# Enigmatisms/AdaPT

Measured on AMD Instinct MI355X. Metric: Msamples/s (W*H*spp/s), unidirectional MIS path tracing, higher is better.
Workload: dtype f32

## Files before the change

adapt_amd/_lib.py:

```python
from __future__ import annotations

import ctypes as C
import os

_HERE = os.path.dirname(os.path.abspath(__file__))
LIB_PATHS = {"fast": os.environ.get("ADAPT_MI_LIB") or os.path.join(_HERE, "libadapt_mi.so"),
             "exact": os.environ.get("ADAPT_MI_LIB_EXACT") or os.path.join(_HERE, "libadapt_mi_exact.so")}
_variant = "exact" if os.environ.get("APT_EXACT", "0") not in ("", "0") else "fast"
LIB_PATH = LIB_PATHS[_variant]

f32p = C.POINTER(C.c_float)
i32p = C.POINTER(C.c_int32)
u32p = C.POINTER(C.c_uint32)
u8p = C.POINTER(C.c_uint8)
f64p = C.POINTER(C.c_double)
APT_N_KERNELS = 5
KERNEL_NAMES = ("generate", "extend", "shade", "shadow", "finalize")


class AptError(RuntimeError):
    pass


class SceneDesc(C.Structure):
# ... 67 lines not shown
    "apt_get_stats": (C.c_int, [C.c_void_p, C.POINTER(Stats)]),
    "apt_device_ptr": (C.c_int, [C.c_void_p, C.POINTER(C.c_void_p), i32p]),
    "apt_stream": (C.c_int, [C.c_void_p, C.POINTER(C.c_void_p)]),
    "apt_intersect": (C.c_int, [C.c_void_p, C.c_int32, f32p, f32p, i32p, f32p, f32p]),
    "apt_occluded": (C.c_int, [C.c_void_p, C.c_int32, f32p, f32p, f32p, i32p]),
    "apt_rng_stream": (C.c_int, [C.c_int32, C.c_uint32, C.c_uint32, C.c_uint32, C.c_int32, u32p]),
    "apt_bxdf_probe": (C.c_int, [C.c_int32, C.c_int32, i32p, f32p, f32p, C.c_float, C.c_int32, C.c_uint32, f32p]),
    "apt_medium_probe": (C.c_int, [C.c_int32, C.c_int32, i32p, f32p, C.c_int32, f32p, C.c_uint32, f32p]),
    "apt_volume_probe": (C.c_int, [C.c_int32, C.c_int32, i32p, f32p, f32p, C.c_int32, f32p, C.c_uint32, f32p]),
    "apt_emitter_probe": (C.c_int, [C.c_void_p, C.c_int32, f32p, C.c_uint32, f32p]),
    "apt_texture_probe": (C.c_int, [C.c_void_p, C.c_int32, i32p, f32p, f32p]),
    "apt_surface_maps_probe": (C.c_int, [C.c_void_p, C.c_int32, i32p, f32p, f32p]),
    "apt_transient_bin_probe": (C.c_int, [C.c_int32, C.c_int32, f32p, C.c_float, C.c_float, C.c_int32, i32p]),
    "apt_renderer_info": (C.c_int, [C.c_void_p, i32p, i32p, C.POINTER(C.c_int64), i32p, C.POINTER(C.c_char_p), i32p]),
    "apt_renderer_camera_fused": (C.c_int, [C.c_void_p, i32p]),
    "apt_measure_sclk_mhz": (C.c_int, [C.c_int32, f32p]),
    "apt_last_error": (C.c_char_p, []),
    "apt_version": (C.c_char_p, []),
}

_libs = {}


def use(variant: str) -> str:
    global _variant, LIB_PATH
    if variant not in LIB_PATHS:
        raise ValueError(f"unknown build variant {variant!r}")
    prev, _variant = _variant, variant
    LIB_PATH = LIB_PATHS[variant]
    return prev
# ... 36 lines not shown
```

adapt_amd/csrc/api.hip:

```cpp
#include <hip/hip_runtime.h>
#include <chrono>

#include <algorithm>
#include <cmath>
#include <cstdio>
#include <cstdlib>
#include <cstring>
#include <limits>
#include <memory>
#include <string>
#include <vector>

#include "../../include/adapt_mi.h"
#include "bvh_build.hpp"
#include "shade_stage.hpp"
#include "unit_kernels.hpp"
#include "volumetric.hpp"

#define APT_EXPORT extern "C" __attribute__((visibility("default")))

static thread_local std::string g_err;
static int fail(int code, const std::string& msg) { g_err = msg; return code; }
#define HIP_TRY(expr)                                                                              \
    do {                                                                                           \
// ... 164 lines not shown

enum Pipeline { PIPE_STAGED, PIPE_SORTED, PIPE_TRACED, PIPE_VOLUMETRIC };

struct apt_renderer {
    const apt_scene* scene = nullptr;
    apt_render_cfg cfg{};
    Params par{};
    int n_cols = 0, npix = 0, spp_batch = 1;
    int cnt = 0;
    std::vector<Lane> lanes;
    int n_lanes = 1;
    hipStream_t stream() const { return lanes[0].stream; }
    DevBuf accum, scratch, pix_key;
    DevBuf cam_strips;
    int camera_fuse = 0;
    Counters host_counters{};
    int grid_small = 0, grid_trace = 0, nq = APT_MAX_NQ;
    const ShadeVariant* shade = nullptr;
    int trace_mode = TRACE_BVH;
    int trace_nt = BLOCK;
    int trace_items = BLOCK;
    Pipeline pipeline = PIPE_STAGED;
    int dyn_fetch = 0;
    bool tile_ok = false;
    extend_fn extend = nullptr, fix = nullptr;
    int ovf_levels = 0;
    int n_cq = 0;
    int vev_single = 0;
    vev_shade_fn vev_all = nullptr;
    bool vev_live[APT_MAX_CLASSES] = {};
// ... 458 lines not shown
    }
    r->spp_batch = B;
    const int S = c.num_shadow_ray;
    const size_t subcap = subcap_of(B), cap = subcap * nq;
    if (cap >= (1ull << 31)) { return fail(APT_E_INVALID, "apt_renderer_create: batch too large (spp_per_batch * pixels must stay below 2^31)"); }
    Params& p = r->par;
    memcpy(p.cam_r, c.cam_r, sizeof(p.cam_r)); memcpy(p.cam_t, c.cam_t, sizeof(p.cam_t));
    p.inv_focal = c.inv_focal; p.half_w = c.half_w; p.half_h = c.half_h;
    p.W = c.width; p.H = c.height; p.n_cols = r->n_cols; p.npix = r->npix;
    p.band_width = c.band_width; p.rank = c.rank; p.world = c.world_size;
    p.do_crop = c.do_crop; p.sx = c.start_x; p.ex = c.end_x; p.sy = c.start_y; p.ey = c.end_y;
    p.max_bounce = c.max_bounce; p.S = S; p.inv_S = (S > 0) ? 1.f / (float)S : 1.f;
    p.use_rr = c.use_rr; p.use_mis = c.use_mis; p.anti_alias = c.anti_alias; p.stratified = c.stratified; p.two_sides = c.brdf_two_sides;
    p.rr_bounce_th = c.rr_bounce_th; p.rr_threshold = c.rr_threshold; p.seed = c.seed; p.cap = (uint32_t)cap; p.subcap = (uint32_t)subcap; p.nq = r->nq;
    p.inv_ns = 1.f / (float)sc->n_sources; p.inv_ns1 = (sc->n_sources > 1) ? 1.f / (float)(sc->n_sources - 1) : 1.f;
    p.volumetric_flat = c.volumetric ? 1 : 0; p.fix_par = 0;
    p.pix_bits = 0; while ((1u << p.pix_bits) < (uint32_t)r->npix) p.pix_bits++;
    if (((uint64_t)B << p.pix_bits) > (1ull << 32)) { return fail(APT_E_INVALID, "apt_renderer_create: spp_per_batch x pixels does not fit the 32-bit path id"); }
    std::vector<uint32_t> key((size_t)r->npix);
    for (int lp = 0; lp < r->npix; lp++) {
        const int lc = lp / c.height, j = lp % c.height, lb = lc / c.band_width, w_ = lc % c.band_width;
        const int i = (lb * c.world_size + c.rank) * c.band_width + w_;
        key[(size_t)lp] = (uint32_t)(i * c.height + j);
    }
    hipError_t e_ = upload(r->pix_key, key);
    if (e_ != hipSuccess) { return fail(APT_E_HIP, std::string("upload pix_key: ") + hipGetErrorString(e_)); }
    p.pix_key = r->pix_key.as<uint32_t>();
    return APT_OK;
}

static int small_scene_sweep(const apt_renderer* r) { return (r->tile_ok && r->scene->max_obj_prims >= APT_SWEEP_LIST_MIN) ? TRACE_TILE : TRACE_SWEEP; }
// ... 82 lines not shown
    cf.inv_focal = c.inv_focal; cf.half_w = c.half_w; cf.half_h = c.half_h;
    cf.width = c.width; cf.height = c.height; cf.n_cols = owned_columns(c); cf.band_width = c.band_width; cf.rank = c.rank; cf.world = c.world_size;
    return cf;
}
static int make_camera_strips(apt_renderer* r) {
    if (r->pipeline != PIPE_TRACED) return APT_OK;
    const apt_scene* sc = r->scene;
    const bool cull = !(getenv("APT_CAMERA_CULL") && atoi(getenv("APT_CAMERA_CULL")) == 0);
    std::vector<uint64_t> masks;
    if (apt::camera_strips(sc->h_prims.data(), sc->n_prims, sc->h_flat_recs, sc->h_flat_tab, sc->h_flat_counts, cam_film(r->cfg), cull, masks) != 0)
        return fail(APT_E_INVALID, "apt_renderer_create: camera strip lists: bad record or film");
    hipError_t e = upload(r->cam_strips, masks);
    if (e != hipSuccess) return fail(APT_E_HIP, std::string("upload camera strip lists: ") + hipGetErrorString(e));
    const bool want = !(getenv("APT_CAMERA_FUSE") && atoi(getenv("APT_CAMERA_FUSE")) == 0);
    r->camera_fuse = (want && !r->adaptive && !r->par.do_crop && r->par.max_bounce >= 1 && r->shade->traced_cam != nullptr) ? 1 : 0;
    return APT_OK;
}

APT_EXPORT int apt_camera_strips(const float* prims, int32_t n_prims, const int32_t* obj_info, int32_t n_objects, const apt_render_cfg* cfg, int32_t cull,
                                 uint64_t* masks, int32_t masks_cap, int32_t* n_strips, int32_t* n_pairs) {
    if (!prims || !obj_info || !cfg || n_prims <= 0 || n_objects <= 0 || !n_strips || !n_pairs) return fail(APT_E_INVALID, "apt_camera_strips: bad argument");
    apt_render_cfg c = *cfg;
    if (c.world_size <= 0) { c.world_size = 1; c.rank = 0; }
    if (c.band_width <= 0) c.band_width = c.width;
    if (c.width <= 0 || c.height <= 0 || c.rank < 0 || c.rank >= c.world_size || owned_columns(c) <= 0) return fail(APT_E_INVALID, "apt_camera_strips: bad film or rank");
    std::vector<float> st, tb; int cn[7];
    if (apt::build_flat(prims, n_prims, obj_info, n_objects, nullptr, st, tb, cn) != 0) return fail(APT_E_INVALID, "apt_camera_strips: obj_info range outside the primitive array");
    std::vector<uint64_t> m;
    if (apt::camera_strips(prims, n_prims, st, tb, cn, cam_film(c), cull != 0, m) != 0) return fail(APT_E_INVALID, "apt_camera_strips: bad record or film");
    *n_strips = (int32_t)m.size();
// ... 406 lines not shown
static int render_surface(apt_renderer* r, int32_t n_spp) {
    const DevScene& sc = r->scene->dev;
    const int nq = r->nq;
    int done = 0, batch = 0;
    hipEvent_t prev_fin = nullptr;
    const int batch_cap = lane_batch(r, n_spp);
    while (done < n_spp) {
        const int B = (n_spp - done < batch_cap) ? (n_spp - done) : batch_cap;
        Lane& ln = r->lanes[(size_t)(batch % r->n_lanes)];
        hipStream_t st = ln.stream;
        const Queues& q = ln.q;
        Counters* cnt = ln.cnt();
        Params p = r->par; p.cnt_base = r->cnt; p.spp_batch = B;
        const size_t total = (size_t)r->npix * (size_t)B;
        if (int rc = begin_batch(r, ln)) return rc;
#if APT_FAST
        if (r->pipeline == PIPE_TRACED) {
            const unsigned long long* strips = r->cam_strips.as<unsigned long long>();
            int cur = 0, b0 = 0;
            if (r->camera_fuse) {
                { LaunchTimer t(r, APT_K_SHADE, st); hipLaunchKernelGGL(r->shade->traced_cam, dim3(grid_for(total, r->grid_small, nq)), dim3(BLOCK), 0, st, sc, p, q, cnt, strips); }
                { LaunchTimer t(r, APT_K_SHADE, st); hipLaunchKernelGGL(r->shade->traced, dim3(r->grid_fix), dim3(BLOCK), 0, st, sc, p, q, cnt, 0, 0); }
                cur = 1; b0 = 1;
            } else {
                LaunchTimer t(r, APT_K_GENERATE, st);
                if (r->adaptive) hipLaunchKernelGGL(k_generate_trace_ad, dim3(grid_for(total, r->grid_small, 1)), dim3(BLOCK), 0, st, sc, p, q, cnt, (const uint8_t*)r->aq.active, strips);
                else hipLaunchKernelGGL(k_generate_trace, dim3(grid_for(total, r->grid_small, 1)), dim3(BLOCK), 0, st, sc, p, q, cnt, strips);
            }
            for (int b = b0; b < p.max_bounce; b++) {
                { LaunchTimer t(r, APT_K_SHADE, st); hipLaunchKernelGGL(r->shade->traced, dim3(grid_for(total, r->grid_small, nq)), dim3(BLOCK), 0, st, sc, p, q, cnt, cur, b); }
// ... 422 lines not shown
    }
    std::vector<unsigned long long> h((size_t)n_waves * 2);
    HIP_TRY(hipMemcpy(h.data(), out.p, h.size() * 8, hipMemcpyDeviceToHost));
    std::vector<double> r;
    for (int w = 0; w < n_waves; w++) if (h[2 * (size_t)w + 1] > 0) r.push_back(100.0 * (double)h[2 * (size_t)w] / (double)h[2 * (size_t)w + 1]);
    if (r.empty()) return fail(APT_E_STATE, "apt_measure_sclk_mhz: the wall clock did not advance");
    std::nth_element(r.begin(), r.begin() + r.size() / 2, r.end());
    *mhz = (float)r[r.size() / 2];
    return APT_OK;
}
APT_EXPORT int apt_renderer_camera_fused(const apt_renderer* r, int32_t* out) {
    if (!r || !out) return fail(APT_E_INVALID, "apt_renderer_camera_fused: null argument");
    *out = r->camera_fuse;
    return APT_OK;
}
APT_EXPORT int apt_renderer_info(const apt_renderer* r, int32_t* spp_batch, int32_t* n_subqueues, int64_t* queue_bytes, int32_t* lds_bytes, const char** shade_variant, int32_t* trace_mode) {
    if (!r) return fail(APT_E_INVALID, "apt_renderer_info: null handle");
    if (spp_batch) *spp_batch = r->spp_batch;
    if (n_subqueues) *n_subqueues = r->nq;
    if (queue_bytes) *queue_bytes = (int64_t)r->lanes[0].pool.bytes * (int64_t)r->lanes.size();
    if (lds_bytes) *lds_bytes = (int32_t)r->lds_bytes;
    if (shade_variant) *shade_variant = r->shade_name.c_str();
    if (trace_mode) *trace_mode = r->trace_mode;
    return APT_OK;
}
```

adapt_amd/csrc/shade_stage.hpp:

```cpp
#pragma once
#include "stages.hpp"

APT_D float ti_fmod(float a, float b) { float q = floorf(a / b); return a - b * q; }
APT_D f3 mix3(f3 a, f3 b, float t) { return a * (1.0f - t) + b * t; }
APT_D f3 texture_query(const DevScene& sc, int map, int obj, float u, float v) {
    const int* ti_ = sc.tex_i + 15 * obj + 5 * map; const float* tf = sc.tex_f + 6 * obj + 2 * map;
    const float w = (float)ti_[3], h = (float)ti_[4];
    const float scaled_u = ti_fmod((u * tf[0]) * w, w - 1.f), scaled_v = ti_fmod((v * tf[1]) * h, h - 1.f);
    float floor_u = floorf(scaled_u), floor_v = floorf(scaled_v);
    const float ratio_u = fmaxf(scaled_u - floor_u, 0.f), ratio_v = fmaxf(scaled_v - floor_v, 0.f);
    floor_u = fminf(fmaxf(floor_u, 0.f), w - 1.f); floor_v = fminf(fmaxf(floor_v, 0.f), h - 1.f);
    const float ceil_u = fminf(floor_u + 1.f, w - 1.f), ceil_v = fminf(floor_v + 1.f, h - 1.f);
    const int fu = (int)(floor_u + (float)ti_[1]), fv = (int)(floor_v + (float)ti_[2]), cu = (int)(ceil_u + (float)ti_[1]), cv = (int)(ceil_v + (float)ti_[2]);
    const float* img = sc.atlas[map]; const int W = sc.atlas_w[map];
    const float* r0 = img + (size_t)fv * W * 3; const float* r1 = img + (size_t)cv * W * 3;
    const f3 q_ff = ld3(r0 + 3 * fu), q_cf = ld3(r0 + 3 * cu), q_fc = ld3(r1 + 3 * fu), q_cc = ld3(r1 + 3 * cu);
    return mix3(mix3(q_ff, q_cf, ratio_u), mix3(q_fc, q_cc, ratio_u), ratio_v);
}
APT_D bool get_uv_item(const DevScene& sc, int map, int obj, int prim, float bu, float bv, f3& out) {
    if (sc.atlas[map] == nullptr || !(sc.tex_i[15 * obj + 5 * map] > -255)) return false;
    const float* uv = sc.uvs + 6 * prim;
    const float w0 = 1.f - bu - bv;
    const float gu = (uv[2] * bu + uv[4] * bv) + uv[0] * w0, gv = (uv[3] * bu + uv[5] * bv) + uv[1] * w0;
    out = texture_query(sc, map, obj, gu, gv);
// ... 55 lines not shown
    const bool need_uv = sc.has_vn || sc.tex_i != nullptr;
    for (uint32_t base = 0; base < n_def; base += 64u) {
        const uint32_t li = base + lane_id(); const bool valid = li < n_def;
        const uint32_t lj = valid ? li : n_def - 1u;
        const uint32_t io = (q.tr_stage_top ? qbase + p.subcap - n_def + lj : (uint32_t)ncls * p.cap + qbase + lj) << 4;
        const float4 ra = ldq(q.tr[cur][0], io), rb = ldq(q.tr[cur][1], io), rc = ldq(q.tr[cur][2], io), rd = ldq(q.tr[cur][3], io);
        const f3 o = mk3(ra.x, ra.y, ra.z), d = mk3(rb.x, rb.y, rb.z);
        HitRec r0, r1; r0.t = r1.t = 1e7f; r0.prim = r1.prim = -1; r0.u = r0.v = r1.u = r1.v = 0.f;
        int c0, c1;
        flat_closest2(sc.flat, sc.sweep, sc.prim_class, o, d, o, d, r0, r1, c0, c1);
        if (valid && r0.prim >= 0) {
            const int oc = ncls > 1 ? c0 : 0;
            const uint32_t pos = atomicAdd(&cnt->n_tr[bounce % 3][oc][sq * CNT_PAD], 1u);
            const uint32_t slot = (uint32_t)oc * p.cap + qbase + pos, so = slot << 4;
            stq(q.tr[cur][0], so, make_float4(ra.x, ra.y, ra.z, r0.t));
            stq(q.tr[cur][1], so, make_float4(rb.x, rb.y, rb.z, __uint_as_float((__float_as_uint(rb.w) & ~0xffu) | (uint32_t)r0.prim)));
            stq(q.tr[cur][2], so, rc); stq(q.tr[cur][3], so, rd);
            if (need_uv) { float2 uv_; uv_.x = r0.u; uv_.y = r0.v; stq(q.tr_uv[cur], slot << 3, uv_); }
        } else if (valid && !(rd.x == 0.f && rd.y == 0.f && rd.z == 0.f)) {
            const uint32_t id = __float_as_uint(rc.w), lp_ = id & ((1u << p.pix_bits) - 1u), s_ = id >> p.pix_bits;
            add_radiance(q.L, p.cap, (s_ * (uint32_t)p.npix + lp_) << 2, mk3(rd.x, rd.y, rd.z), true);
        }
    }
    uint32_t t_lit = 0;
    for (uint32_t base = 0; base < n_sh; base += 64u) {
        const uint32_t li = base + lane_id(); const bool valid = li < n_sh;
        const uint32_t io = (sh_qbase + (valid ? li : n_sh - 1u)) << 2;
        const f3 o = ld3q(q.sh_o, q.sh_cap, io), d = ld3q(q.sh_d, q.sh_cap, io), c = ld3q(q.sh_c, q.sh_cap, io);
        const float dist = ldq(q.sh_tmax, io); const uint32_t slot = ldq(q.sh_id, io);
        bool occ, occ_b;
        const float lim = shadow_limit(dist);
        flat_any2(sc.flat, sc.sweep, o, d, o, d, lim, lim, occ, occ_b);
        const bool weird = !(isfinite(c.x) && isfinite(c.y) && isfinite(c.z));
        const bool add = valid && (!occ || weird);
        for (unsigned long long m = __ballot(add); m != 0ull; m &= m - 1ull) {
            if ((int)lane_id() == __ffsll((long long)m) - 1) add_radiance(q.L, p.cap, slot, occ ? c * 0.f : c, true);
// ... 154 lines not shown
    uint32_t pf_pm = 0;
    auto prefetch_prim = [&](uint32_t b) { pf_pm = ldq(reinterpret_cast<const uint32_t*>(trB), ((qbase + min(b + threadIdx.x, n - 1u)) << 4) + 12u); };
    if (PFP && n > 0) prefetch_prim(sl.first);
    for (uint32_t base = sl.first; base < n; base += sl.stride) {
        APT_ARGS_PHASE();
        const uint32_t pos = base + threadIdx.x, idx = qbase + pos;
        bool alive = pos < n;
        const uint32_t cu_pm = pf_pm;
        float4 cu_ra = make_float4(0.f, 0.f, 0.f, 0.f), cu_rb = cu_ra;
        if (PFP) { const int rp = max(tr_prim(cu_pm), 0); cu_ra = (A_->sc).prim_shade[2 * rp]; cu_rb = (A_->sc).prim_shade[2 * rp + 1]; prefetch_prim(base + sl.stride); }
        Vertex vx; vertex_reset(vx);
        Rng rng; rng_init(rng, 0u, 0u, 0u, 0u);
        f3 Lc = splat3(0.f);
        bool entry = alive;
        float ray_pdf = 1.f;
        if constexpr (CAM) {
            const uint32_t w = (uint32_t)__builtin_amdgcn_readfirstlane((int)(pos >> 6)) * (uint32_t)(A_->p).nq + (uint32_t)sl.q;
            const uint32_t id_ = w * 64u + lane_id();
            const bool valid = alive && id_ < cam_total;
            f3 dir = mk3(0.f, 0.f, 1.f);
            uint32_t draws = 0;
            uint32_t jitter_tail[2] = {0u, 0u};
            if (valid) {
                const uint32_t lp = id_ % (uint32_t)(A_->p).npix, s = id_ / (uint32_t)(A_->p).npix;
                int i, j; local_to_global((A_->p), lp, i, j);
                for (int pl = 0; pl < (A_->p).l_planes; pl++) stL((A_->q).L, (A_->p).cap, (id_ << 2) | (uint32_t)pl, splat3(0.f));
                dir = camera_ray_dir((A_->p), i, j, s, draws, WINDOW ? jitter_tail : nullptr);
                vx.id = (s << (A_->p).pix_bits) | lp;
            }
            if (draws) atomicAdd(&s_draws[threadIdx.x >> 6], draws);
            const f3 cam_o = mk3((A_->p).cam_t[0], (A_->p).cam_t[1], (A_->p).cam_t[2]);
            float c_t = 0.f; int c_run = -1, c_idx = -1;
            if (__any(valid)) c_idx = flat_closest1<true>((A_->sc).flat, cam_o, dir, 1e7f, c_t, c_run, camera_strip_mask((A_->p), strips, w));
            const bool c_defer = valid && (c_run >= 0 || flat_needs_cull((A_->sc).flat, dir));
            HitRec hr; hr.t = 1e7f; hr.prim = -1; hr.u = hr.v = 0.f;
            int hit_cls = 0;
            if (valid && !c_defer && c_idx >= 0) flat_resolve((A_->sc).flat, c_idx, c_t, cam_o, dir, hr, hit_cls);
            { const uint32_t nv = wave_count(valid); t_samples += nv; t_extend += nv; }
            if (__any(c_defer)) {
                const int ncls = (A_->q).tr_ncls;
                const uint32_t dpos = wave_append(c_defer, &cnt->n_tr[0][ncls][sl.q * CNT_PAD]);
// ... 11 lines not shown
            entry = valid && !c_defer;
            alive = entry && hr.prim >= 0;
            if (alive) {
                vx.o = cam_o; vx.d = dir; vx.thr = splat3(1.f);
                f3 rec_kd; float2 uv; uv.x = hr.u; uv.y = hr.v;
                build_hit((A_->sc), hr.prim, hr.t, uv.x, uv.y, vx.o, vx.d, vx.it, vx.hit_light, rec_kd);
                alive = open_vertex<BM, SM, TEX>(A_, vx, rng, hr.prim, rec_kd, tr_meta(tr_pack(hr.prim, draws, false), 0u), ray_pdf, uv, 0, WINDOW ? jitter_tail : nullptr);
            }
        }
        if (!CAM && alive && bounce > 0) { const float4 dd = ldq(trD, idx << 4); Lc = mk3(dd.x, dd.y, dd.z); if (SM & APT_SRC_AREA) ray_pdf = dd.w; }
        if (!CAM && alive) {
            const float4 a = ldq(trA, idx << 4), b_ = ldq(trB, idx << 4), c = ldq(trC, idx << 4);
            vx.o = mk3(a.x, a.y, a.z); vx.d = mk3(b_.x, b_.y, b_.z); vx.thr = mk3(c.x, c.y, c.z); vx.id = __float_as_uint(c.w);
            const uint32_t pm = PFP ? cu_pm : __float_as_uint(b_.w);
            const int prim = tr_prim(pm);
            if (prim < 0) alive = false;
            else {
                f3 rec_kd; float2 uv; uv.x = uv.y = 0.f;
                if ((A_->sc).has_vn || (TEX && (A_->sc).tex_i != nullptr)) uv = ldq((A_->q).tr_uv[cur], idx << 3);
                if (PFP) build_hit_rec((A_->sc), cu_ra, cu_rb, prim, a.w, uv.x, uv.y, vx.o, vx.d, vx.it, vx.hit_light, rec_kd);
                else build_hit((A_->sc), prim, a.w, uv.x, uv.y, vx.o, vx.d, vx.it, vx.hit_light, rec_kd);
                alive = open_vertex<BM, SM, TEX>(A_, vx, rng, prim, rec_kd, tr_meta(pm, (uint32_t)bounce), ray_pdf, uv, bounce);
            }
        }
        tl.shade += wave_count(alive);
#ifdef APT_NEAR_STATS
        t_near += wave_count(alive && bounce > 0 && vx.it.min_depth < 2e-3f);
#endif
        if (alive) vx.hit_point = vx.d * vx.it.min_depth + vx.o;

// ... 13 lines not shown
                if (!__any(f.want && f.src != e0)) occ_e = e0;
            }
        }
        APT_ARGS_PHASE();
        bool cont = false, is_spec = false;
        f3 new_d = mk3(0.f, 1.f, 0.f);
        float new_pdf = 1.f;
        if (alive) {
            new_d = emit_and_scatter<BM, SM>(A_, vx, rng, new_pdf, is_spec, [&](f3 add) { Lc = Lc + add; });
            cont = (bounce + 1) < (A_->p).max_bounce;
        }
        if (rng.draw != vx.draw0) atomicAdd(&s_draws[threadIdx.x >> 6], rng.draw - vx.draw0);
        APT_ARGS_PHASE();
        float tr_t = 0.f; int tr_hit = -1; float tr_u = 0.f, tr_v = 0.f; int tr_q = -1;
        TrAppend tr_app; tr_app.raw = 0u; tr_app.rank = 0u;
        {
            int tr_idx = -1, tr_run = -1, hit_cls = 0;
            if (__any(cont)) tr_idx = flat_closest1((A_->sc).flat, vx.hit_point, new_d, 1e7f, tr_t, tr_run);
            const bool tr_defer = cont && (tr_run >= 0 || flat_needs_cull((A_->sc).flat, new_d));
            t_extend += wave_count(cont);
            cont = cont && (tr_idx >= 0 || tr_defer);
            if (cont && !tr_defer) { HitRec hr; flat_resolve((A_->sc).flat, tr_idx, tr_t, vx.hit_point, new_d, hr, hit_cls); tr_hit = hr.prim; tr_u = hr.u; tr_v = hr.v; }
            tr_q = !cont ? -1 : (tr_defer ? 1 : 0);
            { const Append a_ = append_issue(tr_q == 0, next_counter); tr_app.raw = a_.raw; tr_app.rank = rank_in(a_.m); }
        }
        APT_ARGS_PHASE();
        {
            const bool defer = f.want && flat_needs_cull((A_->sc).flat, f.dir);
            bool occ = false;
            if (__any(f.want && !defer)) {
                const FlatList ls = (occ_e >= 0) ? flat_occ_list((A_->sc).flat, occ_e) : flat_full_list((A_->sc).flat);
                occ = flat_any1(ls, vx.hit_point, f.dir, shadow_limit(f.dist));
            }
            if (__any(defer)) {
                const uint32_t spos = wave_append(defer, &cnt->n_fix_sh[cur][sl.q * CNT_PAD]);
                if (defer && spos < (A_->q).sh_subcap) { const uint32_t so = (sh_qbase + spos) << 2; shadow_store((A_->q), so, vx.hit_point, f.dir, f.dist, f.contrib); stq((A_->q).sh_id, so, vx.l_off); }
            }
            const bool traced = f.want && !defer;
            if (traced) {
                const bool weird = !(isfinite(f.contrib.x) && isfinite(f.contrib.y) && isfinite(f.contrib.z));
                if (!occ || weird) Lc = Lc + (occ ? f.contrib * 0.f : f.contrib);
            }
            t_traced += wave_count(f.want); t_lit += wave_count(traced && !occ);
        }
        uint32_t npos = (uint32_t)__builtin_amdgcn_readlane((int)tr_app.raw, 0) + tr_app.rank;
        if (__any(tr_q == 1)) { const uint32_t dpos = wave_append(tr_q == 1, next_counter + APT_MAX_NQ * CNT_PAD); if (tr_q == 1) npos = dpos; }
        if (cont) {
            const uint32_t slot = (tr_q == 1) ? qbase + (A_->p).subcap - 1u - npos : qbase + npos, so = slot << 4;
            stq((A_->q).tr[nxt][0], so, make_float4(vx.hit_point.x, vx.hit_point.y, vx.hit_point.z, tr_t));
            stq((A_->q).tr[nxt][1], so, make_float4(new_d.x, new_d.y, new_d.z, __uint_as_float(tr_pack(tr_hit, rng.draw, is_spec))));
            stq((A_->q).tr[nxt][2], so, make_float4(vx.thr.x, vx.thr.y, vx.thr.z, __uint_as_float(vx.id)));
            stq((A_->q).tr[nxt][3], so, make_float4(Lc.x, Lc.y, Lc.z, new_pdf));
            if ((A_->sc).has_vn || (A_->sc).tex_i != nullptr) { float2 uv_; uv_.x = tr_u; uv_.y = tr_v; stq((A_->q).tr_uv[nxt], slot << 3, uv_); }
        }
        if (!cont && entry && !(Lc.x == 0.f && Lc.y == 0.f && Lc.z == 0.f)) {
            const uint32_t lp_ = vx.id & ((1u << (A_->p).pix_bits) - 1u), s_ = vx.id >> (A_->p).pix_bits;
            add_radiance((A_->q).L, (A_->p).cap, (s_ * (uint32_t)(A_->p).npix + lp_) << 2, Lc, true);
        }
    }
    flush_uniform(t_traced, &cnt->stats[sl.q][ST_SHADOW_TRACED]); flush_uniform(t_lit, &cnt->stats[sl.q][ST_LIT]);
    flush_uniform(t_extend, &cnt->stats[sl.q][ST_EXTEND]);
    if (CAM) flush_uniform(t_samples, &cnt->stats[sl.q][ST_SAMPLES]);
    tally_flush(tl, s_draws, cnt, sl.q);
#ifdef APT_NEAR_STATS
    flush_uniform(t_near, &cnt->stats[sl.q][14]);
#endif
}
#endif
template <int BM, int SM, int TEX, bool CQ, bool TR = false>
APT_D void shade_staged(args3_ptr A0, Counters* cnt, const ShadeIn& in, int cur, int bounce, TransQ tq = TransQ{}) {
    const ShadeArgs3* A_ = args_fresh(A0);
    const int nxt = cur ^ 1;
// ... 172 lines not shown
```

adapt_amd/csrc/stages.hpp:

```cpp
#pragma once
#include <hip/hip_runtime.h>

#include "rng.hpp"
#include "shading.hpp"
#include "traverse.hpp"
#include "vec.hpp"

struct DevMedium {
    int type;
    float ior;
    f3 u_s, u_a, u_e, par, pdf;
};
struct DevVolume {
    int type, xres, yres, zres;
    f3 albedo, trans, mini, maxi, majorant, pdf;
    f3 inv_r0, inv_r1, inv_r2;
    DevMedium ph;
    const float* grid;
};
struct DevScene {
    DevBvh bvh;
    SweepScene sweep;
    FlatScene flat;
    const float* normals;
// ... 28 lines not shown
    int use_rr, use_mis, anti_alias, stratified, two_sides, rr_bounce_th;
    float rr_threshold;
    uint32_t seed;
    int cnt_base, spp_batch;
    uint32_t cap;
    uint32_t subcap;
    int nq;
    uint32_t pix_bits;
    const uint32_t* pix_key;
    float inv_ns, inv_ns1;
    int fix_par;
    int volumetric_flat;
    int nee_vm;
    int l_planes;
    int traced;
    float w_min[3], w_max[3];
};

struct Queues {
    float* ray_o[2]; float* ray_d[2];
    float* hit_t; int* hit_prim; float* hit_u; float* hit_v;
    float4* tr[2][4]; float2* tr_uv[2]; int tr_ncls, tr_stage_top;
    uint32_t* fix_ext; uint32_t* fix_sh;
    float* thr[2]; uint32_t* id[2]; uint32_t* meta[2]; float* pdf[2];
    float* sh_o; float* sh_d; float* sh_tmax; float* sh_c; uint32_t* sh_id;
    uint32_t* sh_walk[2];
    float* L;
    uint32_t sh_cap, sh_subcap;
    float4* cq[4];
    int n_classes;
// ... 28 lines not shown
    uint32_t n_shadow[APT_MAX_NQ * CNT_PAD];
    uint32_t n_walk[8][APT_MAX_NQ * CNT_PAD];
    uint32_t n_cls[8][APT_MAX_NQ * CNT_PAD];
    uint32_t n_fix_ext[2][APT_MAX_NQ * CNT_PAD];
    uint32_t n_fix_sh[2][APT_MAX_NQ * CNT_PAD];
    uint32_t n_work[2][APT_MAX_NQ * CNT_PAD];
    uint32_t n_tr[3][8 + 1][APT_MAX_NQ * CNT_PAD];
    uint32_t fix_claim[APT_MAX_NQ * CNT_PAD];
    uint32_t fix_done[APT_MAX_NQ * CNT_PAD];
    unsigned long long stats[APT_MAX_NQ][16];
#ifdef APT_WALK_STATS
    unsigned long long wdbg[2][8];
#endif
};

APT_D uint32_t pack_meta(uint32_t draw, uint32_t bounce, bool spec) { return (draw & 0xffffu) | ((bounce & 0xffu) << 16) | (spec ? (1u << 24) : 0u); }

#define BLOCK 256
#define TR_NO_PRIM 0xffu
APT_D uint32_t tr_pack(int prim, uint32_t draw, bool spec) { return (prim < 0 ? TR_NO_PRIM : (uint32_t)prim) | ((draw & 0xffffu) << 8) | (spec ? (1u << 24) : 0u); }
APT_D int tr_prim(uint32_t pm) { return ((pm & 0xffu) == TR_NO_PRIM) ? -1 : (int)(pm & 0xffu); }
APT_D uint32_t tr_meta(uint32_t pm, uint32_t bounce) { return pack_meta(pm >> 8, bounce, ((pm >> 24) & 1u) != 0u); }
#ifndef APT_EXCLUSIVE_L
#define APT_EXCLUSIVE_L(p) ((p).S == 1 || (p).l_planes == (p).S)
#endif

struct LdsPlan { int stack_depth; uint2* ovf; int ovf_stride; };
extern __shared__ float4 s_dyn[];
typedef __attribute__((address_space(3))) float lds_f;
APT_D TravStack make_stack(const LdsPlan& plan) {
    TravStack ts;
    ts.lds = (lds_u2*)(reinterpret_cast<grp_t*>(s_dyn)) + threadIdx.x;
    ts.stride = BLOCK; ts.k = plan.stack_depth; ts.ovf_stride = plan.ovf_stride;
    ts.ovf = plan.ovf ? (glb_u2*)(reinterpret_cast<grp_t*>(plan.ovf) + (blockIdx.x * blockDim.x + threadIdx.x)) : (glb_u2*)nullptr;
    ts.lut = (lds_u8*)nullptr;
    return ts;
}
APT_D TravStack make_walk_stack(const LdsPlan& plan) {
    TravStack ts = make_stack(plan);
    ts.lut = (lds_u8*)(reinterpret_cast<float*>(s_dyn) + (size_t)plan.stack_depth * BLOCK * 2 + 6 * BLOCK);
    fill_permute_lut(ts.lut);
    __syncthreads();
    return ts;
}

APT_D uint32_t lane_id() { return threadIdx.x & 63u; }
APT_D float* L_slot(float* L, uint32_t cap, uint32_t code) { return L + (size_t)(code & 3u) * 4 * cap + (size_t)(code & ~3u); }
APT_D f3 ldL(float* L, uint32_t cap, uint32_t code) { const float4 v = *reinterpret_cast<const float4*>(L_slot(L, cap, code)); return mk3(v.x, v.y, v.z); }
APT_D void stL(float* L, uint32_t cap, uint32_t code, f3 v) { *reinterpret_cast<float4*>(L_slot(L, cap, code)) = make_float4(v.x, v.y, v.z, 0.f); }
APT_D void add_radiance(float* L, uint32_t cap, uint32_t code, f3 c, bool exclusive) {
    if (exclusive) { const f3 a = ldL(L, cap, code); stL(L, cap, code, mk3(a.x + c.x, a.y + c.y, a.z + c.z)); }
    else { float* p_ = L_slot(L, cap, code); atomicAdd(p_, c.x); atomicAdd(p_ + 1, c.y); atomicAdd(p_ + 2, c.z); }
}
APT_D float shadow_limit(float dist) { return (dist > 0.0f) ? dist - 1e-4f : 1e7f; }
APT_D bool non_finite(f3 c) { return !(isfinite(c.x) && isfinite(c.y) && isfinite(c.z)); }
APT_D uint32_t rank_in(unsigned long long m) { return __builtin_amdgcn_mbcnt_hi((uint32_t)(m >> 32), __builtin_amdgcn_mbcnt_lo((uint32_t)m, 0u)); }
APT_D uint32_t wave_append(bool flag, uint32_t* counter) {
    unsigned long long m = __ballot(flag);
    uint32_t base = 0;
    if (lane_id() == 0 && m) base = atomicAdd(counter, (uint32_t)__popcll(m));
    base = (uint32_t)__builtin_amdgcn_readlane((int)base, 0);
    return base + rank_in(m);
}

struct Append { unsigned long long m; uint32_t raw; };
APT_D Append append_issue(bool flag, uint32_t* counter) {
    Append a; a.m = __ballot(flag); a.raw = 0;
// ... 780 lines not shown
```

adapt_amd/renderer.py:

```python
from __future__ import annotations

import ctypes as C
import time
from typing import List, Optional

import numpy as np

from . import _lib
from .scene_pack import FlatScene, RenderConfig, make_config, pack_scene
from .tiles import TilePlan

__all__ = ["Renderer", "VolumeRenderer", "DeviceScene", "bxdf_probe", "medium_probe", "volume_probe", "rng_stream", "adaptive_config", "adaptive_segments", "relative_error"]

ADAPTIVE_DEFAULTS = {"min_spp": 64, "step": 32}
TRAVERSAL_NAMES = dict(enumerate(("bvh", "sweep", "tile", "flat")))


def adaptive_config(adaptive) -> Optional[dict]:
    if adaptive is None or adaptive is False:
        return None
    if not isinstance(adaptive, dict):
        raise TypeError("adaptive must be None or a dict {'threshold': t, 'min_spp': 64, 'step': 32}")
    unknown = set(adaptive) - {"threshold", "min_spp", "step"}
    if unknown:
# ... 395 lines not shown
    def info(self) -> dict:
        b, nq, lds, tm = C.c_int32(0), C.c_int32(0), C.c_int32(0), C.c_int32(0)
        qb = C.c_int64(0)
        name = C.c_char_p()
        _lib.check(self.lib.apt_renderer_info(self.handle, C.byref(b), C.byref(nq), C.byref(qb), C.byref(lds), C.byref(name), C.byref(tm)), "apt_renderer_info", self.lib)
        return {"spp_per_batch": b.value, "n_subqueues": nq.value, "queue_bytes": qb.value, "lds_bytes": lds.value,
                "shade_variant": name.value.decode() if name.value else "",
                "traversal": TRAVERSAL_NAMES.get(tm.value, str(tm.value)), "arithmetic": self.arithmetic,
                "sampling": "adaptive" if self.adaptive else "uniform", **({"adaptive": dict(self.adaptive)} if self.adaptive else {})}

    def camera_fused(self) -> bool:
        f = C.c_int32(0)
        _lib.check(self.lib.apt_renderer_camera_fused(self.handle, C.byref(f)), "apt_renderer_camera_fused", self.lib)
        return bool(f.value)

    def get_check_point(self) -> dict:
        return {"w": self.w, "h": self.h, "crop_x": self.crop_x, "crop_y": self.crop_y, "crop_rx": self.crop_rx,
                "crop_ry": self.crop_ry, "focal": self.focal, "num_objects": self.num_objects, "num_prims": self.num_prims,
                "cam_orient": np.array(self.cam_orient), "src_num": self.src_num, "cam_t": np.array(self.cam_t),
                "accumulation": self.color.to_numpy(), "counter": self._cnt,
                **({"transient_bins": self.tile_transient()} if self.n_bins else {}),
                **(self._adaptive_check_point() if self.adaptive else {})}

    _ADAPTIVE_KEYS = ("adaptive", "sample_counts", "moments", "active")

    def _adaptive_check_point(self) -> dict:
        n, act = self.tile_sample_counts(with_mask=True)
        return {"adaptive": dict(self.adaptive), "sample_counts": n, "moments": self.tile_moments(), "active": act}

    def load_check_point(self, check_point: dict):
# ... 46 lines not shown
```

include/adapt_mi.h:

```cpp
#ifndef ADAPT_MI_H
#define ADAPT_MI_H

#include <stdint.h>

#ifdef __cplusplus
extern "C" {
#endif

#define APT_OK            0
#define APT_E_INVALID    -1
#define APT_E_NO_DEVICE  -2
#define APT_E_HIP        -3
#define APT_E_NOMEM      -4
#define APT_E_STATE      -5

typedef struct apt_bvh apt_bvh;
typedef struct apt_scene apt_scene;
typedef struct apt_renderer apt_renderer;

typedef struct apt_scene_desc {
    int32_t n_prims, n_objects, n_sources, has_vertex_normal;
    const float*   prims;
    const float*   normals;
    const float*   v_normals;
// ... 108 lines not shown
int apt_occluded(apt_renderer*, int32_t n, const float* o, const float* d, const float* tmax, int32_t* occ_out);
int apt_rng_stream(int32_t device, uint32_t pixel, uint32_t seed, uint32_t sample, int32_t n, uint32_t* out);
int apt_bxdf_probe(int32_t device, int32_t n, const int32_t* bxdf_i, const float* bxdf_f, const float* dirs12,
                   float world_ior, int32_t do_sample, uint32_t seed, float* out);
int apt_texture_probe(const apt_scene*, int32_t n, const int32_t* map_obj, const float* uv, float* out3);
int apt_surface_maps_probe(const apt_scene*, int32_t n, const int32_t* prim_first, const float* bary, float* out7);
int apt_medium_probe(int32_t device, int32_t n, const int32_t* med_i, const float* med_f, int32_t mode, const float* in7,
                     uint32_t seed, float* out8);
int apt_volume_probe(int32_t device, int32_t n, const int32_t* vol_i, const float* vol_f, const float* vol_grid, int32_t mode,
                     const float* in10, uint32_t seed, float* out8);
int apt_emitter_probe(const apt_scene*, int32_t n, const float* in11, uint32_t seed, float* out12);
int apt_transient_bin_probe(int32_t device, int32_t n, const float* t, float min_time, float interval, int32_t n_bins, int32_t* out);
int apt_renderer_info(const apt_renderer*, int32_t* spp_batch, int32_t* n_subqueues, int64_t* queue_bytes,
                      int32_t* lds_bytes, const char** shade_variant, int32_t* trace_mode);
int apt_renderer_camera_fused(const apt_renderer*, int32_t* fused);

int apt_measure_sclk_mhz(int32_t device, float* mhz);

const char* apt_last_error(void);
const char* apt_version(void);

#ifdef __cplusplus
}
#endif
#endif
```

Baseline: 6126.

## Skip radiance pre-zeroing by tracking path liveness bit and storing L once

Camera rays no longer zero the per-sample radiance planes up front when camera fusion is active. Instead, a new live bit in the packed path word records whether the L slot has been written yet. Terminating paths then store their radiance directly, or read-add-write only if the slot is live, and deferred shadow rays zero the slot first. This removes the initial L zeroing stores and the later read-modify-write for paths that end without prior contributions, at the cost of extra bit bookkeeping and a more fragile invariant on L initialisation.

```diff
diff --git a/adapt_amd/_lib.py b/adapt_amd/_lib.py
--- a/adapt_amd/_lib.py
+++ b/adapt_amd/_lib.py
@@ -105,6 +105,8 @@
     "apt_transient_bin_probe": (C.c_int, [C.c_int32, C.c_int32, f32p, C.c_float, C.c_float, C.c_int32, i32p]),
     "apt_renderer_info": (C.c_int, [C.c_void_p, i32p, i32p, C.POINTER(C.c_int64), i32p, C.POINTER(C.c_char_p), i32p]),
     "apt_renderer_camera_fused": (C.c_int, [C.c_void_p, i32p]),
+    "apt_renderer_l_store_once": (C.c_int, [C.c_void_p, i32p]),
+    "apt_path_word_probe": (C.c_int, [C.c_int32, C.c_uint32, C.c_int32, C.c_int32, C.c_int32, C.c_uint32, u32p]),
     "apt_measure_sclk_mhz": (C.c_int, [C.c_int32, f32p]),
     "apt_last_error": (C.c_char_p, []),
     "apt_version": (C.c_char_p, []),
diff --git a/adapt_amd/csrc/api.hip b/adapt_amd/csrc/api.hip
--- a/adapt_amd/csrc/api.hip
+++ b/adapt_amd/csrc/api.hip
@@ -202,6 +202,7 @@
     DevBuf accum, scratch, pix_key;
     DevBuf cam_strips;
     int camera_fuse = 0;
+    int l_sentinel = 0;
     Counters host_counters{};
     int grid_small = 0, grid_trace = 0, nq = APT_MAX_NQ;
     const ShadeVariant* shade = nullptr;
@@ -690,7 +691,7 @@
     p.use_rr = c.use_rr; p.use_mis = c.use_mis; p.anti_alias = c.anti_alias; p.stratified = c.stratified; p.two_sides = c.brdf_two_sides;
     p.rr_bounce_th = c.rr_bounce_th; p.rr_threshold = c.rr_threshold; p.seed = c.seed; p.cap = (uint32_t)cap; p.subcap = (uint32_t)subcap; p.nq = r->nq;
     p.inv_ns = 1.f / (float)sc->n_sources; p.inv_ns1 = (sc->n_sources > 1) ? 1.f / (float)(sc->n_sources - 1) : 1.f;
-    p.volumetric_flat = c.volumetric ? 1 : 0; p.fix_par = 0;
+    p.volumetric_flat = c.volumetric ? 1 : 0; p.fix_par = 0; p.l_prezeroed = 1;
     p.pix_bits = 0; while ((1u << p.pix_bits) < (uint32_t)r->npix) p.pix_bits++;
     if (((uint64_t)B << p.pix_bits) > (1ull << 32)) { return fail(APT_E_INVALID, "apt_renderer_create: spp_per_batch x pixels does not fit the 32-bit path id"); }
     std::vector<uint32_t> key((size_t)r->npix);
@@ -803,6 +804,9 @@
     if (e != hipSuccess) return fail(APT_E_HIP, std::string("upload camera strip lists: ") + hipGetErrorString(e));
     const bool want = !(getenv("APT_CAMERA_FUSE") && atoi(getenv("APT_CAMERA_FUSE")) == 0);
     r->camera_fuse = (want && !r->adaptive && !r->par.do_crop && r->par.max_bounce >= 1 && r->shade->traced_cam != nullptr) ? 1 : 0;
+    const bool store_once = !(getenv("APT_L_STORE_ONCE") && atoi(getenv("APT_L_STORE_ONCE")) == 0);
+    r->par.l_prezeroed = (r->camera_fuse && store_once) ? 0 : 1;
+    r->l_sentinel = (getenv("APT_L_SENTINEL") && atoi(getenv("APT_L_SENTINEL")) != 0) ? 1 : 0;
     return APT_OK;
 }
 
@@ -1239,6 +1243,10 @@
         Params p = r->par; p.cnt_base = r->cnt; p.spp_batch = B;
         const size_t total = (size_t)r->npix * (size_t)B;
         if (int rc = begin_batch(r, ln)) return rc;
+        if (r->l_sentinel && !p.l_prezeroed) {
+            const float big = 1e30f; int bits; memcpy(&bits, &big, 4);
+            unchain(r, st); HIP_TRY(hipMemsetD32Async((hipDeviceptr_t)q.L, bits, (size_t)4 * p.cap * (size_t)p.l_planes, st));
+        }
 #if APT_FAST
         if (r->pipeline == PIPE_TRACED) {
             const unsigned long long* strips = r->cam_strips.as<unsigned long long>();
@@ -1691,6 +1699,17 @@
     *out = r->camera_fuse;
     return APT_OK;
 }
+APT_EXPORT int apt_renderer_l_store_once(const apt_renderer* r, int32_t* out) {
+    if (!r || !out) return fail(APT_E_INVALID, "apt_renderer_l_store_once: null argument");
+    *out = r->par.l_prezeroed ? 0 : 1;
+    return APT_OK;
+}
+APT_EXPORT int apt_path_word_probe(int32_t prim, uint32_t draw, int32_t spec, int32_t live, int32_t new_prim, uint32_t bounce, uint32_t* out) {
+    if (!out || new_prim < 0 || new_prim >= (int32_t)TR_NO_PRIM) return fail(APT_E_INVALID, "apt_path_word_probe: bad argument");
+    const uint32_t pm = tr_pack(prim, draw, spec != 0, live != 0);
+    out[0] = pm; out[1] = (uint32_t)tr_prim(pm); out[2] = tr_meta(pm, bounce); out[3] = tr_live(pm) ? 1u : 0u; out[4] = tr_rehit(pm, new_prim);
+    return APT_OK;
+}
 APT_EXPORT int apt_renderer_info(const apt_renderer* r, int32_t* spp_batch, int32_t* n_subqueues, int64_t* queue_bytes, int32_t* lds_bytes, const char** shade_variant, int32_t* trace_mode) {
     if (!r) return fail(APT_E_INVALID, "apt_renderer_info: null handle");
     if (spp_batch) *spp_batch = r->spp_batch;
diff --git a/adapt_amd/csrc/shade_stage.hpp b/adapt_amd/csrc/shade_stage.hpp
--- a/adapt_amd/csrc/shade_stage.hpp
+++ b/adapt_amd/csrc/shade_stage.hpp
@@ -93,12 +93,12 @@
             const uint32_t pos = atomicAdd(&cnt->n_tr[bounce % 3][oc][sq * CNT_PAD], 1u);
             const uint32_t slot = (uint32_t)oc * p.cap + qbase + pos, so = slot << 4;
             stq(q.tr[cur][0], so, make_float4(ra.x, ra.y, ra.z, r0.t));
-            stq(q.tr[cur][1], so, make_float4(rb.x, rb.y, rb.z, __uint_as_float((__float_as_uint(rb.w) & ~0xffu) | (uint32_t)r0.prim)));
+            stq(q.tr[cur][1], so, make_float4(rb.x, rb.y, rb.z, __uint_as_float(tr_rehit(__float_as_uint(rb.w), r0.prim))));
             stq(q.tr[cur][2], so, rc); stq(q.tr[cur][3], so, rd);
             if (need_uv) { float2 uv_; uv_.x = r0.u; uv_.y = r0.v; stq(q.tr_uv[cur], slot << 3, uv_); }
-        } else if (valid && !(rd.x == 0.f && rd.y == 0.f && rd.z == 0.f)) {
+        } else if (valid) {
             const uint32_t id = __float_as_uint(rc.w), lp_ = id & ((1u << p.pix_bits) - 1u), s_ = id >> p.pix_bits;
-            add_radiance(q.L, p.cap, (s_ * (uint32_t)p.npix + lp_) << 2, mk3(rd.x, rd.y, rd.z), true);
+            end_path(q.L, p.cap, (s_ * (uint32_t)p.npix + lp_) << 2, mk3(rd.x, rd.y, rd.z), p.l_prezeroed != 0 || tr_live(__float_as_uint(rb.w)));
         }
     }
     uint32_t t_lit = 0;
@@ -283,6 +283,7 @@
         f3 Lc = splat3(0.f);
         bool entry = alive;
         float ray_pdf = 1.f;
+        bool live = false;
         if constexpr (CAM) {
             const uint32_t w = (uint32_t)__builtin_amdgcn_readfirstlane((int)(pos >> 6)) * (uint32_t)(A_->p).nq + (uint32_t)sl.q;
             const uint32_t id_ = w * 64u + lane_id();
@@ -293,7 +294,7 @@
             if (valid) {
                 const uint32_t lp = id_ % (uint32_t)(A_->p).npix, s = id_ / (uint32_t)(A_->p).npix;
                 int i, j; local_to_global((A_->p), lp, i, j);
-                for (int pl = 0; pl < (A_->p).l_planes; pl++) stL((A_->q).L, (A_->p).cap, (id_ << 2) | (uint32_t)pl, splat3(0.f));
+                if ((A_->p).l_prezeroed) for (int pl = 0; pl < (A_->p).l_planes; pl++) stL((A_->q).L, (A_->p).cap, (id_ << 2) | (uint32_t)pl, splat3(0.f));
                 dir = camera_ray_dir((A_->p), i, j, s, draws, WINDOW ? jitter_tail : nullptr);
                 vx.id = (s << (A_->p).pix_bits) | lp;
             }
@@ -335,6 +336,7 @@
             vx.o = mk3(a.x, a.y, a.z); vx.d = mk3(b_.x, b_.y, b_.z); vx.thr = mk3(c.x, c.y, c.z); vx.id = __float_as_uint(c.w);
             const uint32_t pm = PFP ? cu_pm : __float_as_uint(b_.w);
             const int prim = tr_prim(pm);
+            live = tr_live(pm);
             if (prim < 0) alive = false;
             else {
                 f3 rec_kd; float2 uv; uv.x = uv.y = 0.f;
@@ -378,6 +380,7 @@
         APT_ARGS_PHASE();
         float tr_t = 0.f; int tr_hit = -1; float tr_u = 0.f, tr_v = 0.f; int tr_q = -1;
         TrAppend tr_app; tr_app.raw = 0u; tr_app.rank = 0u;
+        bool live_next = live;
         {
             int tr_idx = -1, tr_run = -1, hit_cls = 0;
             if (__any(cont)) tr_idx = flat_closest1((A_->sc).flat, vx.hit_point, new_d, 1e7f, tr_t, tr_run);
@@ -399,6 +402,14 @@
             if (__any(defer)) {
                 const uint32_t spos = wave_append(defer, &cnt->n_fix_sh[cur][sl.q * CNT_PAD]);
                 if (defer && spos < (A_->q).sh_subcap) { const uint32_t so = (sh_qbase + spos) << 2; shadow_store((A_->q), so, vx.hit_point, f.dir, f.dist, f.contrib); stq((A_->q).sh_id, so, vx.l_off); }
+                if (!(A_->p).l_prezeroed) {
+                    if (defer && cont && !live) {
+                        float zero = 0.f;
+                        asm volatile("" : "+v"(zero));
+                        *reinterpret_cast<float4*>(L_slot((A_->q).L, (A_->p).cap, vx.l_off)) = make_float4(zero, zero, zero, zero);
+                    }
+                    live_next = live || defer;
+                }
             }
             const bool traced = f.want && !defer;
             if (traced) {
@@ -412,14 +423,14 @@
         if (cont) {
             const uint32_t slot = (tr_q == 1) ? qbase + (A_->p).subcap - 1u - npos : qbase + npos, so = slot << 4;
             stq((A_->q).tr[nxt][0], so, make_float4(vx.hit_point.x, vx.hit_point.y, vx.hit_point.z, tr_t));
-            stq((A_->q).tr[nxt][1], so, make_float4(new_d.x, new_d.y, new_d.z, __uint_as_float(tr_pack(tr_hit, rng.draw, is_spec))));
+            stq((A_->q).tr[nxt][1], so, make_float4(new_d.x, new_d.y, new_d.z, __uint_as_float(tr_pack(tr_hit, rng.draw, is_spec, live_next))));
             stq((A_->q).tr[nxt][2], so, make_float4(vx.thr.x, vx.thr.y, vx.thr.z, __uint_as_float(vx.id)));
             stq((A_->q).tr[nxt][3], so, make_float4(Lc.x, Lc.y, Lc.z, new_pdf));
             if ((A_->sc).has_vn || (A_->sc).tex_i != nullptr) { float2 uv_; uv_.x = tr_u; uv_.y = tr_v; stq((A_->q).tr_uv[nxt], slot << 3, uv_); }
         }
-        if (!cont && entry && !(Lc.x == 0.f && Lc.y == 0.f && Lc.z == 0.f)) {
+        if (!cont && entry) {
             const uint32_t lp_ = vx.id & ((1u << (A_->p).pix_bits) - 1u), s_ = vx.id >> (A_->p).pix_bits;
-            add_radiance((A_->q).L, (A_->p).cap, (s_ * (uint32_t)(A_->p).npix + lp_) << 2, Lc, true);
+            end_path((A_->q).L, (A_->p).cap, (s_ * (uint32_t)(A_->p).npix + lp_) << 2, Lc, (A_->p).l_prezeroed != 0 || live);
         }
     }
     flush_uniform(t_traced, &cnt->stats[sl.q][ST_SHADOW_TRACED]); flush_uniform(t_lit, &cnt->stats[sl.q][ST_LIT]);
diff --git a/adapt_amd/csrc/stages.hpp b/adapt_amd/csrc/stages.hpp
--- a/adapt_amd/csrc/stages.hpp
+++ b/adapt_amd/csrc/stages.hpp
@@ -66,6 +66,7 @@
     int nee_vm;
     int l_planes;
     int traced;
+    int l_prezeroed;
     float w_min[3], w_max[3];
 };
 
@@ -124,13 +125,16 @@
 #endif
 };
 
-APT_D uint32_t pack_meta(uint32_t draw, uint32_t bounce, bool spec) { return (draw & 0xffffu) | ((bounce & 0xffu) << 16) | (spec ? (1u << 24) : 0u); }
+APT_HD uint32_t pack_meta(uint32_t draw, uint32_t bounce, bool spec) { return (draw & 0xffffu) | ((bounce & 0xffu) << 16) | (spec ? (1u << 24) : 0u); }
 
 #define BLOCK 256
 #define TR_NO_PRIM 0xffu
-APT_D uint32_t tr_pack(int prim, uint32_t draw, bool spec) { return (prim < 0 ? TR_NO_PRIM : (uint32_t)prim) | ((draw & 0xffffu) << 8) | (spec ? (1u << 24) : 0u); }
-APT_D int tr_prim(uint32_t pm) { return ((pm & 0xffu) == TR_NO_PRIM) ? -1 : (int)(pm & 0xffu); }
-APT_D uint32_t tr_meta(uint32_t pm, uint32_t bounce) { return pack_meta(pm >> 8, bounce, ((pm >> 24) & 1u) != 0u); }
+#define TR_LIVE (1u << 25)
+APT_HD uint32_t tr_pack(int prim, uint32_t draw, bool spec, bool live = false) { return (prim < 0 ? TR_NO_PRIM : (uint32_t)prim) | ((draw & 0xffffu) << 8) | (spec ? (1u << 24) : 0u) | (live ? TR_LIVE : 0u); }
+APT_HD int tr_prim(uint32_t pm) { return ((pm & 0xffu) == TR_NO_PRIM) ? -1 : (int)(pm & 0xffu); }
+APT_HD bool tr_live(uint32_t pm) { return (pm & TR_LIVE) != 0u; }
+APT_HD uint32_t tr_rehit(uint32_t pm, int prim) { return (pm & ~0xffu) | (uint32_t)prim; }
+APT_HD uint32_t tr_meta(uint32_t pm, uint32_t bounce) { return pack_meta(pm >> 8, bounce, ((pm >> 24) & 1u) != 0u); }
 #ifndef APT_EXCLUSIVE_L
 #define APT_EXCLUSIVE_L(p) ((p).S == 1 || (p).l_planes == (p).S)
 #endif
@@ -161,6 +165,11 @@
 APT_D void add_radiance(float* L, uint32_t cap, uint32_t code, f3 c, bool exclusive) {
     if (exclusive) { const f3 a = ldL(L, cap, code); stL(L, cap, code, mk3(a.x + c.x, a.y + c.y, a.z + c.z)); }
     else { float* p_ = L_slot(L, cap, code); atomicAdd(p_, c.x); atomicAdd(p_ + 1, c.y); atomicAdd(p_ + 2, c.z); }
+}
+APT_D void end_path(float* L, uint32_t cap, uint32_t code, f3 c, bool add) {
+    f3 a = splat3(0.f);
+    if (add) { if (c.x == 0.f && c.y == 0.f && c.z == 0.f) return; a = ldL(L, cap, code); }
+    stL(L, cap, code, mk3(a.x + c.x, a.y + c.y, a.z + c.z));
 }
 APT_D float shadow_limit(float dist) { return (dist > 0.0f) ? dist - 1e-4f : 1e7f; }
 APT_D bool non_finite(f3 c) { return !(isfinite(c.x) && isfinite(c.y) && isfinite(c.z)); }
diff --git a/adapt_amd/renderer.py b/adapt_amd/renderer.py
--- a/adapt_amd/renderer.py
+++ b/adapt_amd/renderer.py
@@ -433,6 +433,11 @@
         _lib.check(self.lib.apt_renderer_camera_fused(self.handle, C.byref(f)), "apt_renderer_camera_fused", self.lib)
         return bool(f.value)
 
+    def l_store_once(self) -> bool:
+        f = C.c_int32(0)
+        _lib.check(self.lib.apt_renderer_l_store_once(self.handle, C.byref(f)), "apt_renderer_l_store_once", self.lib)
+        return bool(f.value)
+
     def get_check_point(self) -> dict:
         return {"w": self.w, "h": self.h, "crop_x": self.crop_x, "crop_y": self.crop_y, "crop_rx": self.crop_rx,
                 "crop_ry": self.crop_ry, "focal": self.focal, "num_objects": self.num_objects, "num_prims": self.num_prims,
diff --git a/include/adapt_mi.h b/include/adapt_mi.h
--- a/include/adapt_mi.h
+++ b/include/adapt_mi.h
@@ -146,6 +146,8 @@
 int apt_renderer_info(const apt_renderer*, int32_t* spp_batch, int32_t* n_subqueues, int64_t* queue_bytes,
                       int32_t* lds_bytes, const char** shade_variant, int32_t* trace_mode);
 int apt_renderer_camera_fused(const apt_renderer*, int32_t* fused);
+int apt_renderer_l_store_once(const apt_renderer*, int32_t* once);
+int apt_path_word_probe(int32_t prim, uint32_t draw, int32_t spec, int32_t live, int32_t new_prim, uint32_t bounce, uint32_t* out);
 
 int apt_measure_sclk_mhz(int32_t device, float* mhz);
 
```

After: 6159 (median of 3 runs). Within noise of the previous version (+0.5%).
